# mateomarin/two_towers

Measured on AMD Instinct MI355X. Metric: training pairs/sec at global batch=8192, 1/2/4/8 GPUs; MRR@10 match, higher is better.
Workload: dtype bf16; 1 GPU; BASELINE configs[2]: EnhancedTwoTowerModel(300, 256), seq_len 64, batch 8192 per GPU, bf16, hard-negative mining k=5 + margin 0.2, dropout 0.1, Adam; global_batch=8192, seq_len=64, hidden=256, embedding_dim=300, parallelism=dp1, loss=hardneg_margin

## Files before the change

include/tt_hip.h:

```cpp
#ifndef TT_HIP_H
#define TT_HIP_H
#include <stdint.h>

#ifdef __cplusplus
extern "C" {
#endif

#define TT_OK 0
#define TT_EINVAL 1000
#define TT_DT_F32 0
#define TT_DT_BF16 1

const char* tt_version(void);
const char* tt_last_error(void);
int tt_set_option(const char* name, int value);
int tt_get_option(const char* name, int* value);

int tt_embed_gather(int dtype, const void* table, long vocab, int ep, const int32_t* ids, long n,
                    void* out, void* stream);

int tt_pack_rows(int dtype, const float* src, long n, int e, int ep, void* out, void* stream);
typedef struct {
  const float* src;
  const float* src2;
// ... 3 lines not shown
  int dst_bf16;
} tt_pack_job;
int tt_pack_multi(const tt_pack_job* jobs, int njobs, void* stream);

int tt_cast(int dtype, const float* x, long n, void* y, void* stream);

int tt_colsum(const float* x, long rows, int cols, long ld, float* out, int accumulate, void* stream);

typedef struct {
  const void* a[4];
  const void* b[4];
  void* c[4];
  const float* bias[4];
  int bshift[4];
  const void* a_hi[4];
  int a_split;
  uint32_t drop_row0;
} tt_gemm_batch;

int tt_gemm(int dtype, int out_dtype, int a_kouter, int b_kouter, int m, int n, int k,
            const tt_gemm_batch* batch, int nbatch, long lda, long ldb, long ldc, float alpha,
            int beta_accum, int relu, int seq_t, uint32_t drop_seed, float drop_p, int splits,
            float* splitk_ws, void* stream);
long tt_gemm_ws_size(int m, int n, int nbatch, int splits);
int tt_gemm_pick_splits(int m, int n, int k, int nbatch);
int tt_gemm_bres_form(int m, int n, int k, int nbatch, long lda, long ldc);

typedef struct {
  const void* g;
  const void* whh;
  const float* bhn;
  void* y;
  void* x1;
  void* save;
  float* hstate;
  int dir;
  uint32_t drop_seed;
  int drop_col0;
  uint32_t drop_row0;
} tt_gru_fwd_rec;

int tt_gru_fwd(int dtype, const tt_gru_fwd_rec* recs, int nrec, int B, int T, int H, long ldg,
               long ldy, float drop_p, void* ws, long ws_bytes, void* stream);
int tt_gru_fwd_launches(int dtype, int T, int H);
long tt_gru_fwd_ws_size(int dtype, int nrec, int B, int T, int H, long ldg, long ldy);
int tt_gru_fwd_launches_for(int dtype, int nrec, int B, int T, int H, long ldg, long ldy);

typedef struct {
  const void* g; const void* whh; const float* bhn;
// ... 120 lines not shown
```

two_towers_amd/_lib.py:

```python
from __future__ import annotations

import contextlib
import ctypes
import os
from ctypes import POINTER, c_float, c_int, c_long, c_uint32, c_void_p

import torch

_HERE = os.path.dirname(os.path.abspath(__file__))
LIB_PATH = os.environ.get("TT_HIP_LIB", os.path.join(_HERE, "lib", "libtt_hip.so"))

DT_F32 = 0
DT_BF16 = 1
TT_EINVAL = 1000


class TTError(RuntimeError):
    pass


class GruTimeoutError(TTError):
    """A column-split GRU forward launch gave up waiting for one of its member workgroups
    (tt_gru_fwd's status word): that launch's outputs are invalid."""

# ... 73 lines not shown


class Head1BwdIO(ctypes.Structure):
    _fields_ = [
        ("x", c_void_p), ("w1", c_void_p), ("ln_g", c_void_p), ("ln_b", c_void_p), ("p1", c_void_p),
        ("mean", c_void_p), ("rstd", c_void_p), ("dout", c_void_p), ("dx", c_void_p), ("dw1", c_void_p),
        ("db1", c_void_p), ("dg", c_void_p), ("dbeta", c_void_p), ("ws", c_void_p),
    ]


_SIGS = {
    "tt_version": (ctypes.c_char_p, []),
    "tt_last_error": (ctypes.c_char_p, []),
    "tt_set_option": (c_int, [ctypes.c_char_p, c_int]),
    "tt_get_option": (c_int, [ctypes.c_char_p, POINTER(c_int)]),
    "tt_embed_gather": (c_int, [c_int, c_void_p, c_long, c_int, c_void_p, c_long, c_void_p, c_void_p]),
    "tt_pack_rows": (c_int, [c_int, c_void_p, c_long, c_int, c_int, c_void_p, c_void_p]),
    "tt_pack_multi": (c_int, [c_void_p, c_int, c_void_p]),
    "tt_cast": (c_int, [c_int, c_void_p, c_long, c_void_p, c_void_p]),
    "tt_colsum": (c_int, [c_void_p, c_long, c_int, c_long, c_void_p, c_int, c_void_p]),
    "tt_gemm": (c_int, [c_int, c_int, c_int, c_int, c_int, c_int, c_int, POINTER(GemmBatch), c_int, c_long,
                        c_long, c_long, c_float, c_int, c_int, c_int, c_uint32, c_float, c_int, c_void_p,
                        c_void_p]),
    "tt_gemm_ws_size": (c_long, [c_int, c_int, c_int, c_int]),
    "tt_gemm_pick_splits": (c_int, [c_int, c_int, c_int, c_int]),
    "tt_gemm_bres_form": (c_int, [c_int, c_int, c_int, c_int, c_long, c_long]),
    "tt_gru_fwd": (c_int, [c_int, POINTER(GruFwdRec), c_int, c_int, c_int, c_int, c_long, c_long, c_float,
                           c_void_p, c_long, c_void_p]),
    "tt_gru_bwd": (c_int, [c_int, POINTER(GruBwdRec), c_int, c_int, c_int, c_int, c_long, c_long, c_long,
                           c_void_p]),
    "tt_gru_bias_rows": (c_int, [c_int]),
    "tt_gru_bwd_launches": (c_int, [c_int, c_int, c_int]),
    "tt_gru_bwd_carry_on_chip": (c_int, [c_int, c_int, c_int]),
    "tt_gru_fwd_launches": (c_int, [c_int, c_int, c_int]),
    "tt_gru_fwd_ws_size": (c_long, [c_int, c_int, c_int, c_int, c_int, c_long, c_long]),
    "tt_gru_fwd_launches_for": (c_int, [c_int, c_int, c_int, c_int, c_int, c_long, c_long]),
    "tt_gru_fwd_infer": (c_int, [c_int, POINTER(GruInferRec), c_int, c_int, c_int, c_int, c_long, c_long, c_long,
                                 c_void_p, c_long, c_void_p]),
    "tt_gru_infer_scratch_size": (c_long, [c_int, c_int, c_int, c_int, c_int]),
    "tt_proj_head_fwd": (c_int, [c_int, POINTER(HeadFwdIO), c_int, c_int, c_int, c_float, c_void_p]),
    "tt_proj_head_bwd": (c_int, [c_int, POINTER(HeadBwdIO), c_int, c_int, c_int, c_float, c_void_p]),
    "tt_proj_head_bwd_ws_size": (c_long, [c_int, c_int, c_int]),
    "tt_proj_head1_fwd": (c_int, [c_int, POINTER(Head1FwdIO), c_long, c_int, c_float, c_float, c_uint32,
                                  c_void_p]),
    "tt_proj_head1_bwd": (c_int, [c_int, POINTER(Head1BwdIO), c_long, c_int, c_float, c_uint32, c_void_p]),
    "tt_proj_head1_bwd_ws_size": (c_long, [c_int, c_long, c_int]),
    "tt_l2norm_fwd": (c_int, [c_int, c_void_p, c_long, c_int, c_float, c_void_p, c_void_p, c_void_p, c_void_p]),
    "tt_l2norm_bwd": (c_int, [c_void_p, c_void_p, c_void_p, c_long, c_int, c_float, c_void_p, c_int, c_void_p]),
    "tt_infonce_fwd": (c_int, [c_int, c_void_p, c_long, c_void_p, c_long, c_int, c_float, c_float, c_long,
# ... 108 lines not shown
```

two_towers_amd/csrc/tt_api.h:

```cpp
#pragma once
#include <hip/hip_runtime.h>
#include <stdio.h>
#include <string.h>

#include "../../include/tt_hip.h"

namespace tt {
void set_error(const char* fmt, ...);

enum Opt {
  OPT_GRU_STEP,
  OPT_GRU_DEPTH,
  OPT_GRU_BWD_ROWS,
  OPT_GRU_BWD_BIG,
  OPT_GRU_BWD_STREAMS,
  OPT_GEMM_PERSIST,
  OPT_GEMM_A3,
  OPT_GEMM_REGSTAGE,
  OPT_GEMM_STREAM_OUT,
  OPT_HN_GEMM,
  OPT_GRU_BWD_PERSIST,
  OPT_GRU_FWD_STEP_ROWS,
  OPT_INFONCE_FLASH,
  OPT_HN_MAP,
  OPT_GEMM_SKEW,
  OPT_GEMM_PERSIST_MAXK,
  OPT_GRU_FWD_XC,
  OPT_GRU_XC_SKIP,
  OPT_GRU_XC_SPINS,
  OPT_GRU_BWD_SKEW,
  OPT_GRU_FWD_SKEW,
  OPT_GEMM_BRES,
  OPT_GRU_XC_COOP,
  OPT_GEMM_BUF,
  OPT_GEMM_ORDER,
  OPT_GRU_STEP_RING,
  OPT_GRU_FWD_XS,
  OPT_HN_SCAN_GEMM,
  OPT_GEMM_IEPI,
  OPT_BRES_ROWS,
  OPT_HN_SCAN_V,
  OPT_GEMM_W4,
  OPT_BRES_FORM,
  OPT_N
};
int opt(Opt o);
int tt_hn_scan_gemm(const void* q, long bq, const void* d, long nd, int h, long label_off, float* cm, long nch,
                    hipStream_t st);
}

#define TT_CHECK_ARG(cond, ...)            \
  do {                                     \
    if (!(cond)) {                         \
      tt::set_error(__VA_ARGS__);          \
      return TT_EINVAL;                    \
    }                                      \
  } while (0)

#define TT_CHECK_LAUNCH(what)                                                        \
  do {                                                                               \
    hipError_t e_ = hipGetLastError();                                               \
    if (e_ != hipSuccess) {                                                          \
      tt::set_error("%s: %s", what, hipGetErrorString(e_));                          \
      return (int)e_;                                                                \
    }                                                                                \
  } while (0)
// ... 18 lines not shown
```

two_towers_amd/csrc/tt_gemm.hip:

```cpp
#include <float.h>
#include <stdarg.h>
#include <stdlib.h>

#include <atomic>
#include <type_traits>

#include "tt_api.h"
#include "tt_gemm_core.h"

namespace tt {
static thread_local char g_err[512];
void set_error(const char* fmt, ...) {
  va_list ap;
  va_start(ap, fmt);
  vsnprintf(g_err, sizeof(g_err), fmt, ap);
  va_end(ap);
}
}

namespace tt {
namespace {
struct OptDef {
  const char* name;
  const char* env;
  int dflt;
};
constexpr OptDef kOpts[OPT_N] = {
    {"gru_step", "TT_GRU_STEP", 0},               {"gru_depth", "TT_GRU_DEPTH", 4},
    {"gru_bwd_rows", "TT_GRU_BWD_ROWS", 0},     {"gru_bwd_big", "TT_GRU_BWD_BIG", 1},
    {"gru_bwd_streams", "TT_GRU_BWD_STREAMS", 2}, {"gemm_persist", "TT_GEMM_PERSIST", 1},
    {"gemm_a3", "TT_GEMM_A3", 1},                 {"gemm_regstage", "TT_GEMM_REGSTAGE", 0},
    {"gemm_stream_out", "TT_GEMM_STREAM_OUT", 1}, {"hn_gemm", "TT_HN_GEMM", 0},
    {"gru_bwd_persist", "TT_GRU_BWD_PERSIST", 1}, {"gru_fwd_step_rows", "TT_GRU_FWD_STEP_ROWS", 0},
    {"infonce_flash", "TT_INFONCE_FLASH", 1},     {"hn_map", "TT_HN_MAP", 2},
    {"gemm_skew", "TT_GEMM_SKEW", 0},             {"gemm_persist_maxk", "TT_GEMM_PERSIST_MAXK", 24},
    {"gru_fwd_xc", "TT_GRU_FWD_XC", 1},           {"gru_xc_skip", "TT_GRU_XC_SKIP", 0},
    {"gru_xc_spins", "TT_GRU_XC_SPINS", 22},      {"gru_bwd_skew", "TT_GRU_BWD_SKEW", 14},
    {"gru_fwd_skew", "TT_GRU_FWD_SKEW", 0},       {"gemm_bres", "TT_GEMM_BRES", 1},
    {"gru_xc_coop", "TT_GRU_XC_COOP", 0},         {"gemm_buf", "TT_GEMM_BUF", 1},
    {"gemm_order", "TT_GEMM_ORDER", 0},           {"gru_step_ring", "TT_GRU_STEP_RING", 4},
    {"gru_fwd_xs", "TT_GRU_FWD_XS", 1},           {"hn_scan_gemm", "TT_HN_SCAN_GEMM", 0},
    {"gemm_iepi", "TT_GEMM_IEPI", 1},             {"bres_rows", "TT_BRES_ROWS", 32},
    {"hn_scan_v", "TT_HN_SCAN_V", 5},             {"gemm_w4", "TT_GEMM_W4", 0},
    {"bres_form", "TT_BRES_FORM", 1},
};
struct OptTable {
  std::atomic<int> v[OPT_N];
  OptTable() {
    for (int i = 0; i < OPT_N; ++i) {
      const char* e = getenv(kOpts[i].env);
      v[i].store(e && *e ? atoi(e) : kOpts[i].dflt, std::memory_order_relaxed);
    }
  }
};
OptTable& opts() {
  static OptTable t;
  return t;
}
int find_opt(const char* name) {
  for (int i = 0; name && i < OPT_N; ++i)
    if (strcmp(name, kOpts[i].name) == 0) return i;
  return -1;
}
}
int opt(Opt o) { return opts().v[o].load(std::memory_order_relaxed); }
}

// ... 17 lines not shown
struct GemmArgs {
  const void* a[4];
  const void* b[4];
  void* c[4];
  const float* bias[4];
  int bshift[4];
  const void* a_hi[4];
  int a_split;
  long lda, ldb, ldc;
  int M, N, K;
  int splits, kt_per_split;
  float alpha;
  int beta, relu, seq_t;
  uint32_t drop_seed, drop_thresh, drop_row0;
  float drop_inv_keep;
  long part_stride;
  int vec_ok;
  int force_regstage;
  int skew;
  int bias_vec_ok;
  int stream_out;
  int walk_g, walk_x;
  int nbatch;
  float* cm;
  long nch, label_off;
};

constexpr int BM = 128, BN = 128;

#ifndef TT_TAIL_SKIP
#define TT_TAIL_SKIP 1
#endif
using ttg::xcd_remap;
#ifndef PERSIST_IEPI
#define PERSIST_IEPI 1
#endif
#ifndef PERSIST_BAL
#define PERSIST_BAL 1
#endif
#ifndef TT_EPI_PAIR
#define TT_EPI_PAIR 1
#endif
#ifndef TT_GEMM_BAL
#define TT_GEMM_BAL true
#endif

// ... 993 lines not shown
              st8(dst, v);
          } else {
            for (int e = 0; e < 8 && gn + e < g.N; ++e) Elt<TO>::st(dst + e, v[e]);
          }
        }
      }
      __builtin_amdgcn_s_barrier();
    }
    if (late && qn < qend) __builtin_amdgcn_s_barrier();
  }
  if constexpr (IE && A3 && !HN && PERSIST_BAL && std::is_same<TO, bf16_t>::value) {
    if (have_prev) {
      iepi(C0{}, C0{});
      iepi(C0{}, C1{});
      iepi(C1{}, C1{});
      iepi(C1{}, C0{});
    }
  }
  if constexpr (A3)
    if (!late) __builtin_amdgcn_s_barrier();
  asm volatile("s_waitcnt vmcnt(0)" ::: "memory");
}

template <typename TO, int V>
__global__ __launch_bounds__(256) void splitk_reduce_kernel(const float* ws, long part_stride, int splits,
                                                            int M, int N, GemmArgs g) {
  const int bi = blockIdx.y;
  const float* P = ws + (long)bi * splits * part_stride;
  TO* C = static_cast<TO*>(g.c[bi]);
  const float* bias = g.bias[bi];
  const long total = (long)M * N / V;
  for (long e = (long)blockIdx.x * 256 + threadIdx.x; e < total; e += (long)gridDim.x * 256) {
    float v[V];
    if constexpr (V == 4) {
      float4 a = make_float4(0.f, 0.f, 0.f, 0.f);
      for (int s = 0; s < splits; ++s) {
        const float4 b = reinterpret_cast<const float4*>(P + (long)s * part_stride)[e];
        a.x += b.x;
        a.y += b.y;
        a.z += b.z;
        a.w += b.w;
      }
      v[0] = a.x, v[1] = a.y, v[2] = a.z, v[3] = a.w;
    } else {
      v[0] = 0.f;
      for (int s = 0; s < splits; ++s) v[0] += P[(long)s * part_stride + e];
    }
    const int m = (int)(e * V / N), n0 = (int)(e * V % N);
#pragma unroll
    for (int u = 0; u < V; ++u) {
      float x = v[u] * g.alpha;
      if (bias) x += bias[n0 + u];
      TO* p = C + (long)m * g.ldc + n0 + u;
      if (g.beta) x += Elt<TO>::ld(p);
      Elt<TO>::st(p, x);
    }
  }
}

template <typename T, typename TO, int TBM, int TBN, int WGM, int WGN, bool DMA, bool A3 = false, bool BUF = false>
int launch_t(int akout, int bkout, bool shift, const GemmArgs& g, long nwg, hipStream_t st) {
  dim3 grid((unsigned)nwg), blk(64 * WGM * WGN);
#define TT_L(AK, BK, SH) \
  hipLaunchKernelGGL((gemm_kernel<T, AK, BK, SH, TO, TBM, TBN, WGM, WGN, DMA, A3, BUF>), grid, blk, 0, st, g)
  if (!akout && !bkout) TT_L(false, false, false);
  else if (!akout && bkout && !shift) TT_L(false, true, false);
  else if (!akout && bkout && shift) TT_L(false, true, true);
  else if (akout && !bkout) TT_L(true, false, false);
  else if (akout && bkout && !shift) TT_L(true, true, false);
  else TT_L(true, true, true);
#undef TT_L
  TT_CHECK_LAUNCH("gemm_kernel");
  return 0;
}

inline bool use_big(int m, int n, long tiles256) { return m >= 256 && n >= 256 && tiles256 >= 256; }
// ... 254 lines not shown
#define TT_WR(n)                                                                   \
  case n:                                                                          \
    if (form == 2)                                                                 \
      hipLaunchKernelGGL((gemm_wreg<n>), grid, blk, 0, st, g, npan, nbatch);       \
    else if (r64)                                                                  \
      hipLaunchKernelGGL((gemm_bres<n, 4>), grid, blk, 0, st, g, npan, nbatch);    \
    else                                                                           \
      hipLaunchKernelGGL((gemm_bres<n, 2>), grid, blk, 0, st, g, npan, nbatch);    \
    break;
      TT_WR(1) TT_WR(2) TT_WR(3) TT_WR(4) TT_WR(5) TT_WR(6) TT_WR(7) TT_WR(8) TT_WR(9) TT_WR(10) TT_BR(11) TT_BR(12)
#undef TT_WR
#undef TT_BR
      default: return false;
    }
    const hipError_t e = hipGetLastError();
    if (e != hipSuccess) {
      tt::set_error("%s: %s", form == 2 ? "gemm_wreg" : "gemm_bres", hipGetErrorString(e));
      *rc = (int)e;
    }
    return true;
  }
}

template <typename T, typename TO>
int launch_gemm(int akout, int bkout, bool shift, GemmArgs& g, int nbatch, hipStream_t st) {
  constexpr int EPC = 16 / (int)sizeof(T);
  {
    int rc = 0;
    if (try_bres<T, TO>(akout, bkout, shift, g, nbatch, st, &rc)) return rc;
  }
  const bool dma = (akout ? g.M % EPC == 0 : g.K % EPC == 0) && (bkout ? g.N % EPC == 0 : g.K % EPC == 0) &&
                   g.force_regstage != 1;
  const long t256 = (long)tt_ceil_div(g.M, 256) * tt_ceil_div(g.N, 256) * nbatch * g.splits;
  const bool persist_ok = tt::opt(tt::OPT_GEMM_PERSIST) != 0;
  const int nk = (g.K * (int)sizeof(T) + ttg::KTB - 1) / ttg::KTB;
  bool buf = tt::opt(tt::OPT_GEMM_BUF) != 0 && g.K % (ttg::KTB / (int)sizeof(T)) == 0;
  {
    const long span = (long)(g.kt_per_split + 2) * (ttg::KTB / (int)sizeof(T)) * (long)sizeof(T);
    if (akout && span * g.lda >= (1L << 32)) buf = false;
    if (bkout && span * g.ldb >= (1L << 32)) buf = false;
    if (shift && g.seq_t % (ttg::KTB / (int)sizeof(T)) != 0) buf = false;
    if (!akout && (long)256 * g.lda * (long)sizeof(T) >= (1L << 31)) buf = false;
    if (!bkout && (long)256 * g.ldb * (long)sizeof(T) >= (1L << 31)) buf = false;
    for (int b = 0; b < 4 && g.a_split > 0; ++b) {
      if (!g.a[b]) continue;
      const long d = (long)((const char*)g.a_hi[b] - (const char*)g.a[b]) / (long)sizeof(T);
      if (d < 0 || d + (g.M - g.a_split) > g.lda) buf = false;
    }
  }
  if constexpr (std::is_same<T, bf16_t>::value && std::is_same<TO, bf16_t>::value) {
    if (tt::opt(tt::OPT_GEMM_W4) && !akout && !bkout && !shift && g.splits == 1 && !g.beta && !g.relu &&
        !g.drop_thresh && g.alpha == 1.f && g.force_regstage == 0 && g.M % 256 == 0 && g.N % 256 == 0 && g.K % 64 == 0 &&
// ... 38 lines not shown
  g.alpha = 1.f;
  g.splits = 1;
  g.kt_per_split = h / 64;
  g.nbatch = 1;
  g.cm = cm;
  g.nch = nch;
  g.label_off = label_off;
  const long ntm = (bq + 255) / 256, ntn = (nd + 255) / 256, ntiles = ntm * ntn;
  TT_CHECK_ARG(ntiles < (1L << 31), "tt_hn_scan_gemm: too many tiles");
  if (ntiles % 256 == 0 && ntn % 4 == 0) {
    g.walk_g = 4;
    g.walk_x = 8;
  }
  hipLaunchKernelGGL((gemm_persist<bf16_t, false, false, false, float, true, true, true>),
                     dim3((unsigned)std::min<long>(ntiles, 256)), dim3(512), 0, st, g, (int)ntiles);
  TT_CHECK_LAUNCH("gemm_persist (hard-negative scan)");
  return 0;
}

extern "C" int tt_gemm_bres_form(int m, int n, int k, int nbatch, long lda, long ldc) {
  return bres_form_for(m, n, k, nbatch, lda, ldc);
}

extern "C" long tt_gemm_ws_size(int m, int n, int nbatch, int splits) {
  (void)m;
  return splits > 1 ? (long)m * n * nbatch * splits : 0;
}

extern "C" int tt_gemm_pick_splits(int m, int n, int k, int nbatch) {
  const bool big = m >= 256 && n >= 256;
  const long tiles = big ? (long)tt_ceil_div(m, 256) * tt_ceil_div(n, 256) * nbatch
                         : (long)tt_ceil_div(m, BM) * tt_ceil_div(n, BN) * nbatch;
  const long target = big ? 512 : 1024;
  if (tiles >= target) return 1;
  const int smax = std::max(1, std::min(64, tt_ceil_div(k, 64) / 8));
  int best = 1;
  double best_eff = 0.0;
  const int s_lo = (int)std::min<long>(smax, std::max<long>(1, target / tiles));
  for (int s = s_lo; s <= std::min<long>(smax, 3 * target / tiles + 1); ++s) {
    const long w = tiles * s;
    const double eff = (double)w / (256.0 * (double)tt_ceil_div(w, 256));
    if (eff > best_eff + 1e-9) { best_eff = eff; best = s; }
  }
  return std::min(best, smax);
}

extern "C" int tt_gemm(int dtype, int out_dtype, int a_kouter, int b_kouter, int m, int n, int k,
                       const tt_gemm_batch* batch, int nbatch, long lda, long ldb, long ldc,
                       float alpha, int beta_accum, int relu, int seq_t, uint32_t drop_seed,
                       float drop_p, int splits, float* splitk_ws, void* stream) {
  TT_CHECK_ARG(dtype == TT_DT_F32 || dtype == TT_DT_BF16, "tt_gemm: bad dtype %d", dtype);
  TT_CHECK_ARG(out_dtype == TT_DT_F32 || out_dtype == dtype, "tt_gemm: bad out_dtype %d", out_dtype);
  TT_CHECK_ARG(nbatch >= 1 && nbatch <= 4, "tt_gemm: nbatch %d not in [1,4]", nbatch);
  TT_CHECK_ARG(m >= 0 && n >= 0 && k >= 0, "tt_gemm: negative dims");
  if (m == 0 || n == 0) return 0;
  const int esz = dtype == TT_DT_BF16 ? 2 : 4;
  const int epc = 16 / esz;
  (void)epc;
  TT_CHECK_ARG((lda * esz) % 16 == 0 && (ldb * esz) % 16 == 0,
               "tt_gemm: leading dimensions must be 16-byte multiples (lda=%ld ldb=%ld)", lda, ldb);
  if (splits < 1) splits = 1;
  TT_CHECK_ARG(splits == 1 || (relu == 0 && drop_p == 0.f), "tt_gemm: split-K excludes relu/dropout");
  TT_CHECK_ARG(splits == 1 || splitk_ws != nullptr, "tt_gemm: split-K needs a workspace");
  TT_CHECK_ARG(drop_p >= 0.f && drop_p < 1.f, "tt_gemm: drop_p %f", drop_p);
  bool shift = false;
  GemmArgs g{};
  for (int b = 0; b < nbatch; ++b) {
    TT_CHECK_ARG(batch->a[b] && batch->b[b] && batch->c[b], "tt_gemm: null operand in batch %d", b);
    TT_CHECK_ARG(((uintptr_t)batch->a[b] | (uintptr_t)batch->b[b]) % 16 == 0,
                 "tt_gemm: operands must be 16-byte aligned (batch %d)", b);
    g.a[b] = batch->a[b];
    g.b[b] = batch->b[b];
    g.c[b] = batch->c[b];
    g.bias[b] = batch->bias[b];
    g.bshift[b] = batch->bshift[b];
    g.a_hi[b] = batch->a_hi[b];
    if (batch->a_split > 0)
      TT_CHECK_ARG(batch->a_hi[b] && (uintptr_t)batch->a_hi[b] % 16 == 0, "tt_gemm: a_hi[%d] null or misaligned", b);
    if (batch->bshift[b] != 0) shift = true;
  }
  TT_CHECK_ARG(!shift || (b_kouter && seq_t > 0), "tt_gemm: bshift needs b_kouter and seq_t");
  TT_CHECK_ARG(batch->a_split >= 0 && (batch->a_split == 0 || (a_kouter && batch->a_split % (16 / esz) == 0)),
               "tt_gemm: a_split %d needs a_kouter and a 16-byte multiple", batch->a_split);
  g.a_split = batch->a_split;
  g.lda = lda; g.ldb = ldb; g.ldc = ldc;
  g.M = m; g.N = n; g.K = k;
  g.alpha = alpha; g.beta = beta_accum; g.relu = relu; g.seq_t = seq_t;
  g.force_regstage = tt::opt(tt::OPT_GEMM_REGSTAGE);
  g.nbatch = nbatch;
  g.skew = tt::opt(tt::OPT_GEMM_SKEW);
  g.drop_seed = drop_seed;
  g.drop_row0 = batch->drop_row0;
  g.drop_thresh = drop_p > 0.f ? (uint32_t)(drop_p * 16777216.0f + 0.5f) : 0u;
  g.drop_inv_keep = drop_p > 0.f ? 1.0f / (1.0f - drop_p) : 1.0f;
  const int nk = tt_ceil_div((long)k * esz, 128);
  if (splits > nk) splits = nk > 0 ? nk : 1;
  g.kt_per_split = nk > 0 ? tt_ceil_div(nk, splits) : 1;
  splits = nk > 0 ? tt_ceil_div(nk, g.kt_per_split) : 1;
  g.splits = splits;
  {
    const int osz = out_dtype == TT_DT_BF16 ? 2 : 4;
    bool ok = (ldc * osz) % 16 == 0;
    for (int b = 0; b < nbatch; ++b) ok = ok && ((uintptr_t)batch->c[b] % 16 == 0);
    g.vec_ok = ok;
    bool bok = true;
    for (int b = 0; b < nbatch; ++b) bok = bok && ((uintptr_t)batch->bias[b] % 16 == 0);
    g.bias_vec_ok = bok;
    g.stream_out = ok && (long)m * n * osz >= (64L << 20) && (long)256 * ldc * osz < (1L << 31);
    g.stream_out = g.stream_out ? tt::opt(tt::OPT_GEMM_STREAM_OUT) : 0;
  }
  hipStream_t st = static_cast<hipStream_t>(stream);
  TT_CHECK_ARG((long)tt_ceil_div(m, 128) * tt_ceil_div(n, 128) * nbatch * splits < (1L << 31), "tt_gemm: too many tiles");

  if (splits > 1) {
    GemmArgs gp = g;
    gp.part_stride = (long)m * n;
    gp.vec_ok = (n % 4 == 0);
    for (int b = 0; b < nbatch; ++b) gp.c[b] = splitk_ws + (long)b * splits * gp.part_stride;
    int rc = dtype == TT_DT_BF16 ? launch_gemm<bf16_t, float>(a_kouter, b_kouter, shift, gp, nbatch, st)
                                 : launch_gemm<float, float>(a_kouter, b_kouter, shift, gp, nbatch, st);
    if (rc) return rc;
    const bool v4 = n % 4 == 0 && (uintptr_t)splitk_ws % 16 == 0;
// ... 19 lines not shown
```

two_towers_amd/csrc/tt_gemm_core.h:

```cpp
#pragma once
#include <type_traits>

#include "tt_common.h"

typedef __bf16 bf16x8v __attribute__((ext_vector_type(8)));
typedef short s16x4 __attribute__((ext_vector_type(4)));
typedef __attribute__((address_space(3))) s16x4 lds_s16x4;

#ifndef TT_PRIO_HALF
#define TT_PRIO_HALF 0
#endif
#ifndef TT_SHIFT_BUF
#define TT_SHIFT_BUF 1
#endif

namespace ttg {

constexpr int KTB = 128;

TT_DEV int kc_off(int row, int c) { return row * KTB + ((c ^ ((row >> 1) & 7)) << 4); }
TT_DEV int ko_v(int k) { return (k & 3) | (((k >> 3) & 1) << 2); }
TT_DEV int ko16_off(int k, int c) { return k * 256 + ((c ^ (ko_v(k) << 1)) << 4); }
TT_DEV int ko32_off_chunk(int k, int c) { return k * 512 + ((c ^ (((k >> 2) & 1) << 2)) << 4); }
TT_DEV int ko32_off_elem(int k, int m) { return k * 512 + ((m ^ (((k >> 2) & 1) << 4)) << 2); }

template <typename T, bool KO, int ROWS>
struct Img {
  static constexpr int BYTES = KO ? (KTB / (int)sizeof(T)) * ROWS * (int)sizeof(T) : ROWS * KTB;
  static constexpr int CHUNKS = BYTES / 16;
  static_assert(!KO || ROWS == 128, "K-outer images are 128 columns wide");
};


template <typename T>
TT_DEV uint4 load_partial(const T* p, int n) {
  union {
    uint4 v;
    T e[16 / sizeof(T)];
  } u;
  u.v = make_uint4(0, 0, 0, 0);
#pragma unroll
  for (int i = 0; i < (int)(16 / sizeof(T)); ++i)
    if (i < n) u.e[i] = p[i];
  return u.v;
}
// ... 59 lines not shown
    const int o0 = ko16_off(k0, cc >> 1) + ((cc & 1) << 3);
    const int o1 = ko16_off(k1, cc >> 1) + ((cc & 1) << 3);
    s16x4 lo = __builtin_amdgcn_ds_read_tr16_b64_v4i16((lds_s16x4*)(img + o0));
    s16x4 hi = __builtin_amdgcn_ds_read_tr16_b64_v4i16((lds_s16x4*)(img + o1));
    uint4 v;
    v.x = (uint32_t)(uint16_t)lo[0] | ((uint32_t)(uint16_t)lo[1] << 16);
    v.y = (uint32_t)(uint16_t)lo[2] | ((uint32_t)(uint16_t)lo[3] << 16);
    v.z = (uint32_t)(uint16_t)hi[0] | ((uint32_t)(uint16_t)hi[1] << 16);
    v.w = (uint32_t)(uint16_t)hi[2] | ((uint32_t)(uint16_t)hi[3] << 16);
    return v;
  } else {
    const int g = lane >> 4;
    const int m = r0 + (lane & 15);
    const int kb = ks * 16 + 4 * g;
    uint4 v;
    v.x = *reinterpret_cast<const uint32_t*>(img + ko32_off_elem(kb + 0, m));
    v.y = *reinterpret_cast<const uint32_t*>(img + ko32_off_elem(kb + 1, m));
    v.z = *reinterpret_cast<const uint32_t*>(img + ko32_off_elem(kb + 2, m));
    v.w = *reinterpret_cast<const uint32_t*>(img + ko32_off_elem(kb + 3, m));
    return v;
  }
}

template <typename T>
TT_DEV f32x4 mma(uint4 a, uint4 b, f32x4 c) {
  if constexpr (sizeof(T) == 2) {
    return __builtin_amdgcn_mfma_f32_16x16x32_bf16(__builtin_bit_cast(bf16x8v, a),
                                                   __builtin_bit_cast(bf16x8v, b), c, 0, 0, 0);
  } else {
    c = __builtin_amdgcn_mfma_f32_16x16x4f32(__uint_as_float(a.x), __uint_as_float(b.x), c, 0, 0, 0);
    c = __builtin_amdgcn_mfma_f32_16x16x4f32(__uint_as_float(a.y), __uint_as_float(b.y), c, 0, 0, 0);
    c = __builtin_amdgcn_mfma_f32_16x16x4f32(__uint_as_float(a.z), __uint_as_float(b.z), c, 0, 0, 0);
    c = __builtin_amdgcn_mfma_f32_16x16x4f32(__uint_as_float(a.w), __uint_as_float(b.w), c, 0, 0, 0);
    return c;
  }
}

template <typename T, bool AKO, bool BKO, int BM, int BN>
struct MainLoop {
  using IA = Img<T, AKO, BM>;
  using IB = Img<T, BKO, BN>;
  static constexpr int STAGE = IA::BYTES + IB::BYTES;
  static constexpr int LDS_BYTES = 2 * STAGE;
  static constexpr int TM = BM / 32, TN = BN / 32;
  static_assert(IA::CHUNKS % 256 == 0 && IB::CHUNKS % 256 == 0, "tile/thread mismatch");

// ... 748 lines not shown
```

two_towers_amd/ops.py:

```python
from __future__ import annotations

import ctypes
from typing import Sequence

import torch

from . import _lib
from ._lib import GemmBatch, call, dtype_code, ptr, stream_ptr


def _esz(dt: torch.dtype) -> int:
    return 2 if dt == torch.bfloat16 else 4


def pad_cols(e: int, dt: torch.dtype) -> int:
    epc = 128 // _esz(dt)
    return (e + epc - 1) // epc * epc


def gemm(a: Sequence[torch.Tensor], b: Sequence[torch.Tensor], c: Sequence[torch.Tensor], *, m: int, n: int,
         k: int, lda: int, ldb: int, ldc: int, a_kouter: bool, b_kouter: bool, dtype: torch.dtype,
         out_dtype: torch.dtype, bias: Sequence[torch.Tensor | None] | None = None,
         bshift: Sequence[int] | None = None, alpha: float = 1.0, accumulate: bool = False,
         relu: bool = False, seq_t: int = 0, drop_seed: int = 0, drop_p: float = 0.0, drop_row0: int = 0,
         splits: int | None = None, a_hi: Sequence[torch.Tensor] | None = None, a_split: int = 0):
    nb = len(a)
    assert 1 <= nb <= 4 and len(b) == nb and len(c) == nb
    bt = GemmBatch()
    for i in range(nb):
        assert a[i].dtype == dtype and b[i].dtype == dtype, (a[i].dtype, b[i].dtype, dtype)
        assert c[i].dtype == out_dtype, (c[i].dtype, out_dtype)
        bt.a[i] = a[i].data_ptr()
        bt.b[i] = b[i].data_ptr()
        bt.c[i] = c[i].data_ptr()
        bt.bias[i] = bias[i].data_ptr() if bias is not None and bias[i] is not None else None
        bt.bshift[i] = bshift[i] if bshift is not None else 0
        if a_split:
            bt.a_hi[i] = a_hi[i].data_ptr()
    bt.a_split = a_split
    bt.drop_row0 = drop_row0 & 0xFFFFFFFF
    lib = _lib.load()
    if splits is None:
        splits = lib.tt_gemm_pick_splits(m, n, k, nb)
    ws = None
    if splits > 1 and not relu and drop_p == 0.0:
        ws = torch.empty(lib.tt_gemm_ws_size(m, n, nb, splits), dtype=torch.float32, device=c[0].device)
    else:
        splits = 1
    call("tt_gemm", dtype_code(dtype), dtype_code(out_dtype), int(a_kouter), int(b_kouter), m, n, k,
         ctypes.byref(bt), nb, lda, ldb, ldc, alpha, int(accumulate), int(relu), seq_t, drop_seed & 0xFFFFFFFF,
         drop_p, splits, ptr(ws), stream_ptr(c[0].device))


def embed_gather(table: torch.Tensor, ids: torch.Tensor, out: torch.Tensor):
    assert ids.dtype == torch.int32 and ids.is_contiguous()
    assert table.dim() == 2 and out.shape[-1] == table.shape[1] and out.dtype == table.dtype
    call("tt_embed_gather", dtype_code(table.dtype), table.data_ptr(), table.shape[0], table.shape[1],
         ids.data_ptr(), ids.numel(), out.data_ptr(), stream_ptr(out.device))


def pack_rows(src: torch.Tensor, out: torch.Tensor):
    assert src.dtype == torch.float32 and src.is_contiguous()
    e = src.shape[-1]
    n = src.numel() // e
    call("tt_pack_rows", dtype_code(out.dtype), src.data_ptr(), n, e, out.shape[-1], out.data_ptr(),
         stream_ptr(out.device))


def cast(x: torch.Tensor, out: torch.Tensor):
    assert x.dtype == torch.float32 and x.is_contiguous() and out.numel() == x.numel()
    call("tt_cast", dtype_code(out.dtype), x.data_ptr(), x.numel(), out.data_ptr(), stream_ptr(out.device))


def colsum(x: torch.Tensor, rows: int, cols: int, ld: int, out: torch.Tensor, accumulate: bool = False):
# ... 30 lines not shown
```

two_towers_amd/towers.py:

```python
from __future__ import annotations

import ctypes
import os
import threading
from dataclasses import dataclass

import torch
import torch.nn.functional as F

from . import _lib, dist, ops, timing
from ._lib import GruBwdRec, GruFwdRec, GruInferRec, HeadBwdIO, HeadFwdIO, call, dtype_code, stream_ptr

PARAMS_PER_TOWER = 22
LN_EPS = 1e-5
HEAD_DT = torch.float32


def gru_param_names():
    names = []
    for layer in (0, 1):
        for sfx in ("", "_reverse"):
            for w in ("weight_ih", "weight_hh", "bias_ih", "bias_hh"):
                names.append(f"{w}_l{layer}{sfx}")
    return names
# ... 406 lines not shown


def _weight_grads(cfg, B, T, dG, Xin, K, ldx, Y, kr=None):
    n, H, dt, dev = cfg.ntowers, cfg.H, cfg.dtype, dG[0].device
    BT = B * T
    dWih = [[_alloc((3 * H, K), torch.float32, dev) for _ in range(2)] for _ in range(n)]
    dWhh = [[_alloc((3 * H, H), torch.float32, dev) for _ in range(2)] for _ in range(n)]
    a_ih, b_ih, c_ih, a_hh, a_hi, b_hh, c_hh, sh = [], [], [], [], [], [], [], []
    for ti in range(n):
        for d in range(2):
            a_ih.append(dG[ti][:, d * 3 * H:])
            b_ih.append(Xin[ti])
            c_ih.append(dWih[ti][d])
            a_hh.append(dG[ti][:, d * 3 * H:])
            a_hi.append(dG[ti][:, 6 * H + d * H:])
            b_hh.append(Y[ti][:, d * H:])
            c_hh.append(dWhh[ti][d])
            sh.append(-1 if d == 0 else 1)
    esz = 2 if dt == torch.bfloat16 else 4
    kr = K if kr is None else kr
    with timing.region("wgrad_ih", 1, 2.0 * 3 * H * kr * BT * 2 * n,
                       float(n * (esz * BT * (6 * H + kr) + 2 * 3 * H * kr * 4))):
        if _WGRAD_T and dt == torch.bfloat16 and 0 < K % 256 <= 128:
            cT = [_alloc((K, 3 * H), torch.float32, dev) for _ in c_ih]
            ops.gemm(b_ih, a_ih, cT, m=K, n=3 * H, k=BT, lda=ldx, ldb=8 * H, ldc=3 * H, a_kouter=True,
                     b_kouter=True, dtype=dt, out_dtype=torch.float32)
            for c, ct in zip(c_ih, cT):
                c.copy_(ct.t())
        else:
            ops.gemm(a_ih, b_ih, c_ih, m=3 * H, n=K, k=BT, lda=8 * H, ldb=ldx, ldc=K, a_kouter=True,
                     b_kouter=True, dtype=dt, out_dtype=torch.float32)
    with timing.region("wgrad_hh", 1, 2.0 * 3 * H * H * BT * 2 * n,
                       float(n * (esz * BT * (6 * H + 2 * H) + 2 * 3 * H * H * 4))):
        ops.gemm(a_hh, b_hh, c_hh, m=3 * H, n=H, k=BT, lda=8 * H, ldb=2 * H, ldc=H, a_kouter=True, b_kouter=True,
                 dtype=dt, out_dtype=torch.float32, bshift=sh, seq_t=T, a_hi=a_hi, a_split=2 * H)
    return dWih, dWhh


class TowersFn(torch.autograd.Function):

    @staticmethod
    def forward(ctx, cfg: TowerCfg, table, group, cache_ok, *args):
        n = cfg.ntowers
        xs, params = args[:n], args[n:]
        _lib.require_gpu(*xs, *params)
        check_gru_status(wait=True)
        dt, E, H, h = cfg.dtype, cfg.E, cfg.H, cfg.h
        dev = xs[0].device
        reset_guard_if_reported(dev)
        B, T = xs[0].shape[0], xs[0].shape[1]
        for x in xs:
# ... 179 lines not shown
```

Baseline: 155,800 pairs/s.

## Add tall-M wgrad GEMM kernel and transposed split-K reduce output

New measurement: 157,400 pairs/s, median of 6. +1.1%, better.

```diff
diff --git a/include/tt_hip.h b/include/tt_hip.h
--- a/include/tt_hip.h
+++ b/include/tt_hip.h
@@ -49,9 +49,15 @@
             const tt_gemm_batch* batch, int nbatch, long lda, long ldb, long ldc, float alpha,
             int beta_accum, int relu, int seq_t, uint32_t drop_seed, float drop_p, int splits,
             float* splitk_ws, void* stream);
+int tt_gemm_ct(int dtype, int out_dtype, int a_kouter, int b_kouter, int m, int n, int k,
+               const tt_gemm_batch* batch, int nbatch, long lda, long ldb, long ldc, float alpha,
+               int beta_accum, int relu, int seq_t, uint32_t drop_seed, float drop_p, int splits,
+               float* splitk_ws, int c_trans, void* stream);
 long tt_gemm_ws_size(int m, int n, int nbatch, int splits);
 int tt_gemm_pick_splits(int m, int n, int k, int nbatch);
 int tt_gemm_bres_form(int m, int n, int k, int nbatch, long lda, long ldc);
+int tt_gemm_tall_form(int dtype, int out_dtype, int a_kouter, int b_kouter, int m, int n, int k, long lda,
+                      long ldb, int splits, int extras);
 
 typedef struct {
   const void* g;
diff --git a/two_towers_amd/_lib.py b/two_towers_amd/_lib.py
--- a/two_towers_amd/_lib.py
+++ b/two_towers_amd/_lib.py
@@ -119,9 +119,13 @@
     "tt_gemm": (c_int, [c_int, c_int, c_int, c_int, c_int, c_int, c_int, POINTER(GemmBatch), c_int, c_long,
                         c_long, c_long, c_float, c_int, c_int, c_int, c_uint32, c_float, c_int, c_void_p,
                         c_void_p]),
+    "tt_gemm_ct": (c_int, [c_int, c_int, c_int, c_int, c_int, c_int, c_int, POINTER(GemmBatch), c_int, c_long,
+                           c_long, c_long, c_float, c_int, c_int, c_int, c_uint32, c_float, c_int, c_void_p,
+                           c_int, c_void_p]),
     "tt_gemm_ws_size": (c_long, [c_int, c_int, c_int, c_int]),
     "tt_gemm_pick_splits": (c_int, [c_int, c_int, c_int, c_int]),
     "tt_gemm_bres_form": (c_int, [c_int, c_int, c_int, c_int, c_long, c_long]),
+    "tt_gemm_tall_form": (c_int, [c_int, c_int, c_int, c_int, c_int, c_int, c_int, c_long, c_long, c_int, c_int]),
     "tt_gru_fwd": (c_int, [c_int, POINTER(GruFwdRec), c_int, c_int, c_int, c_int, c_long, c_long, c_float,
                            c_void_p, c_long, c_void_p]),
     "tt_gru_bwd": (c_int, [c_int, POINTER(GruBwdRec), c_int, c_int, c_int, c_int, c_long, c_long, c_long,
diff --git a/two_towers_amd/csrc/tt_api.h b/two_towers_amd/csrc/tt_api.h
--- a/two_towers_amd/csrc/tt_api.h
+++ b/two_towers_amd/csrc/tt_api.h
@@ -42,6 +42,7 @@
   OPT_HN_SCAN_V,
   OPT_GEMM_W4,
   OPT_BRES_FORM,
+  OPT_WGRAD_TALL,
   OPT_N
 };
 int opt(Opt o);
diff --git a/two_towers_amd/csrc/tt_gemm.hip b/two_towers_amd/csrc/tt_gemm.hip
--- a/two_towers_amd/csrc/tt_gemm.hip
+++ b/two_towers_amd/csrc/tt_gemm.hip
@@ -42,7 +42,7 @@
     {"gru_fwd_xs", "TT_GRU_FWD_XS", 1},           {"hn_scan_gemm", "TT_HN_SCAN_GEMM", 0},
     {"gemm_iepi", "TT_GEMM_IEPI", 1},             {"bres_rows", "TT_BRES_ROWS", 32},
     {"hn_scan_v", "TT_HN_SCAN_V", 5},             {"gemm_w4", "TT_GEMM_W4", 0},
-    {"bres_form", "TT_BRES_FORM", 1},
+    {"bres_form", "TT_BRES_FORM", 1},             {"wgrad_tall", "TT_WGRAD_TALL", 1},
 };
 struct OptTable {
   std::atomic<int> v[OPT_N];
@@ -106,6 +106,7 @@
   int stream_out;
   int walk_g, walk_x;
   int nbatch;
+  int c_trans;
   float* cm;
   long nch, label_off;
 };
@@ -1145,6 +1146,140 @@
   asm volatile("s_waitcnt vmcnt(0)" ::: "memory");
 }
 
+namespace tall {
+constexpr int AW = 8192, AN = 4096;
+constexpr int BOFF = 2 * AW + AN;
+constexpr int SLOT = BOFF + 2 * AW;
+constexpr int NS = 4;
+constexpr int NDMA = SLOT / 1024;
+constexpr int KS = 32;
+}
+
+template <bool HALF>
+__global__ __launch_bounds__(512) void gemm_tall(GemmArgs g, int u0) {
+  using namespace tall;
+  constexpr int NA = HALF ? 5 : 10;
+  __shared__ __attribute__((aligned(16))) char lds[NS * SLOT];
+  const int ntn = (g.N + 255) / 256;
+  const int id = xcd_remap(blockIdx.x, gridDim.x);
+  const int hf = HALF ? id & 1 : 0;
+  const int u = u0 + (HALF ? id >> 1 : id);
+  const int bs = u / ntn, nt = u - bs * ntn;
+  const int bi = bs / g.splits, s = bs - bi * g.splits;
+  const int n0 = nt * 256;
+  const bf16_t* A = static_cast<const bf16_t*>(g.a[bi]);
+  const bf16_t* B = static_cast<const bf16_t*>(g.b[bi]);
+  const int wave = __builtin_amdgcn_readfirstlane(threadIdx.x >> 6), lane = threadIdx.x & 63;
+  const int wr = wave >> 2, wn = (wave & 3) * 64;
+  auto a_sub = [&](int a) { return HALF ? a >> 1 : a / 5; };
+  auto a_col = [&](int a) {
+    if (HALF) return a == 4 ? 32 * hf + 16 * wr : 64 * hf + 32 * wr + 16 * (a & 1);
+    return a % 5 == 4 ? 32 * wr + 16 * (a / 5) : 64 * wr + 16 * (a % 5);
+  };
+
+  f32x4 acc[NA][4];
+#pragma unroll
+  for (int i = 0; i < NA; ++i)
+#pragma unroll
+    for (int j = 0; j < 4; ++j) acc[i][j] = f32x4{0.f, 0.f, 0.f, 0.f};
+
+  const int nk = (g.K * 2 + ttg::KTB - 1) / ttg::KTB;
+  const int kt0 = s * g.kt_per_split;
+  const int kt1 = min(nk, kt0 + g.kt_per_split);
+  if (kt0 < kt1) {
+    const int nst = 2 * (kt1 - kt0);
+    const long k0 = (long)kt0 * 64;
+    const long krows = min((long)g.K, (long)kt1 * 64) - k0;
+    const ttg::tt_rsrc4 ra = ttg::make_rsrc4(A + k0 * g.lda, (uint32_t)(((krows - 1) * g.lda + g.M) * 2));
+    const ttg::tt_rsrc4 rb = ttg::make_rsrc4(B + k0 * g.ldb, (uint32_t)(((krows - 1) * g.ldb + g.N) * 2));
+    const uint32_t da = (uint32_t)(KS * g.lda * 2), db = (uint32_t)(KS * g.ldb * 2);
+    uint32_t voff[5];
+#pragma unroll
+    for (int t = 0; t < 5; ++t) {
+      const int j = wave + 8 * t;
+      long e;
+      if (j < 16) {
+        const int p = (j & 7) * 64 + lane, kl = p >> 4, c = (p & 15) ^ (ttg::ko_v(kl) << 1);
+        e = (long)kl * g.lda + (j >> 3) * 128 + c * 8;
+      } else if (j < 20) {
+        const int p = (j - 16) * 64 + lane, kl = p >> 3, c = (p & 7) ^ (ttg::kon_v(kl) << 1);
+        e = (long)kl * g.lda + 256 + c * 8;
+      } else {
+        const int b = j - 20, p = (b & 7) * 64 + lane, kl = p >> 4, c = (p & 15) ^ (ttg::ko_v(kl) << 1);
+        e = (long)kl * g.ldb + n0 + (b >> 3) * 128 + c * 8;
+      }
+      voff[t] = (uint32_t)(e * 2);
+    }
+    const uint32_t base = __builtin_amdgcn_readfirstlane(ttg::lds_addr_of(lds));
+    const bool a2 = wave < 4;
+    ttg::tt_rsrc4 r2;
+    r2.x = a2 ? ra.x : rb.x;
+    r2.y = a2 ? ra.y : rb.y;
+    r2.z = a2 ? ra.z : rb.z;
+    r2.w = ra.w;
+    const uint32_t d2 = a2 ? da : db;
+    auto issue = [&](int st) {
+      const uint32_t sl = base + (uint32_t)(st & (NS - 1)) * SLOT + (uint32_t)wave * 1024u;
+      const uint32_t sa = (uint32_t)st * da, sb = (uint32_t)st * db;
+      ttg::dma16_buf(ra, voff[0] + sa, 0u, sl);
+      ttg::dma16_buf(ra, voff[1] + sa, 0u, sl + 8 * 1024u);
+      ttg::dma16_buf(r2, voff[2] + (uint32_t)st * d2, 0u, sl + 16 * 1024u);
+      ttg::dma16_buf(rb, voff[3] + sb, 0u, sl + 24 * 1024u);
+      if (a2) ttg::dma16_buf(rb, voff[4] + sb, 0u, sl + 32 * 1024u);
+    };
+    auto step = [&](const char* sl) {
+      uint4 fb[4];
+#pragma unroll
+      for (int j = 0; j < 4; ++j) fb[j] = ttg::frag<bf16_t, true>(sl + BOFF + (wn >> 7) * AW, (wn & 127) + 16 * j, 0);
+#pragma unroll
+      for (int h = 0; h < NA / 5; ++h) {
+        uint4 fa[5];
+#pragma unroll
+        for (int i = 0; i < 4; ++i) fa[i] = ttg::frag<bf16_t, true>(sl + a_sub(5 * h + i) * AW, a_col(5 * h + i), 0);
+        fa[4] = ttg::frag_ko16n(sl + 2 * AW, a_col(5 * h + 4));
+#pragma unroll
+        for (int i = 0; i < 5; ++i)
+#pragma unroll
+          for (int j = 0; j < 4; ++j) acc[5 * h + i][j] = ttg::mma<bf16_t>(fb[j], fa[i], acc[5 * h + i][j]);
+        __builtin_amdgcn_sched_barrier(0);
+      }
+    };
+    issue(0);
+    issue(1);
+    issue(2);
+    for (int st = 0; st < nst; ++st) {
+      if (wave < 4) asm volatile("s_waitcnt vmcnt(10)" ::: "memory");
+      else asm volatile("s_waitcnt vmcnt(8)" ::: "memory");
+      __builtin_amdgcn_s_barrier();
+      issue(st + 3);
+      const char* sl = lds + (st & (NS - 1)) * SLOT;
+      step(sl);
+    }
+    asm volatile("s_waitcnt vmcnt(0)" ::: "memory");
+  }
+
+  const bool partial = g.splits > 1;
+  float* C = partial ? static_cast<float*>(g.c[bi]) + (long)s * g.part_stride : static_cast<float*>(g.c[bi]);
+  const long ldc = partial ? (long)g.N : g.ldc;
+  const int q = lane >> 4, lr = lane & 15;
+#pragma unroll
+  for (int i = 0; i < NA; ++i) {
+    const int gm = (i % 5 < 4 ? 128 * a_sub(i) : 256) + a_col(i) + lr;
+#pragma unroll
+    for (int j = 0; j < 4; ++j) {
+      const int c = n0 + wn + 16 * j + 4 * q;
+      if (gm >= g.M || c >= g.N) continue;
+      float v[4];
+#pragma unroll
+      for (int e = 0; e < 4; ++e) v[e] = partial ? acc[i][j][e] : acc[i][j][e] * g.alpha + 0.f;
+      float* dst = C + (long)gm * ldc + c;
+      if (c + 4 <= g.N && g.vec_ok) *reinterpret_cast<float4*>(dst) = make_float4(v[0], v[1], v[2], v[3]);
+      else
+        for (int e = 0; e < 4 && c + e < g.N; ++e) dst[e] = v[e];
+    }
+  }
+}
+
 template <typename TO, int V>
 __global__ __launch_bounds__(256) void splitk_reduce_kernel(const float* ws, long part_stride, int splits,
                                                             int M, int N, GemmArgs g) {
@@ -1174,7 +1309,7 @@
     for (int u = 0; u < V; ++u) {
       float x = v[u] * g.alpha;
       if (bias) x += bias[n0 + u];
-      TO* p = C + (long)m * g.ldc + n0 + u;
+      TO* p = g.c_trans ? C + (long)(n0 + u) * g.ldc + m : C + (long)m * g.ldc + n0 + u;
       if (g.beta) x += Elt<TO>::ld(p);
       Elt<TO>::st(p, x);
     }
@@ -1475,12 +1610,40 @@
   }
 }
 
+bool tall_form_for(bool bf16_in, bool f32_out, int akout, int bkout, bool plain, int M, int N, long lda, long ldb,
+                   int kt_per_split) {
+  if (tt::opt(tt::OPT_WGRAD_TALL) == 0 || !bf16_in || !f32_out || !akout || !bkout || !plain) return false;
+  if (M <= 256 || M > 320 || M % 8 || N % 8 || N <= 0) return false;
+  if (tt::opt(tt::OPT_GEMM_REGSTAGE) != 0) return false;
+  const long span = ((long)kt_per_split * 64 + 4 * tall::KS) * 2;
+  return span * lda < (1L << 32) && span * ldb < (1L << 32);
+}
+bool gemm_args_plain(const GemmArgs& g, bool shift, int nbatch) {
+  if (shift || g.a_split > 0 || g.beta || g.relu || g.drop_thresh) return false;
+  for (int b = 0; b < nbatch; ++b)
+    if (g.bias[b]) return false;
+  return true;
+}
+
 template <typename T, typename TO>
 int launch_gemm(int akout, int bkout, bool shift, GemmArgs& g, int nbatch, hipStream_t st) {
   constexpr int EPC = 16 / (int)sizeof(T);
   {
     int rc = 0;
     if (try_bres<T, TO>(akout, bkout, shift, g, nbatch, st, &rc)) return rc;
+  }
+  if (tall_form_for(std::is_same<T, bf16_t>::value, std::is_same<TO, float>::value, akout, bkout,
+                    gemm_args_plain(g, shift, nbatch), g.M, g.N, g.lda, g.ldb, g.kt_per_split)) {
+    const long units = (long)tt_ceil_div(g.N, 256) * nbatch * g.splits;
+    const int mode = tt::opt(tt::OPT_WGRAD_TALL);
+    long nfull = units;
+    if (mode == 3) nfull = 0;
+    else if (mode != 2 && units % 256 > 0 && units % 256 <= 128) nfull = units - units % 256;
+    if (nfull > 0) hipLaunchKernelGGL(gemm_tall<false>, dim3((unsigned)nfull), dim3(512), 0, st, g, 0);
+    if (units > nfull)
+      hipLaunchKernelGGL(gemm_tall<true>, dim3((unsigned)(2 * (units - nfull))), dim3(512), 0, st, g, (int)nfull);
+    TT_CHECK_LAUNCH("gemm_tall");
+    return 0;
   }
   const bool dma = (akout ? g.M % EPC == 0 : g.K % EPC == 0) && (bkout ? g.N % EPC == 0 : g.K % EPC == 0) &&
                    g.force_regstage != 1;
@@ -1565,6 +1728,23 @@
   return bres_form_for(m, n, k, nbatch, lda, ldc);
 }
 
+static void split_plan(int k, int esz, int* splits, int* kt_per_split) {
+  const int nk = tt_ceil_div((long)k * esz, 128);
+  int s = *splits < 1 ? 1 : *splits;
+  if (s > nk) s = nk > 0 ? nk : 1;
+  *kt_per_split = nk > 0 ? tt_ceil_div(nk, s) : 1;
+  *splits = nk > 0 ? tt_ceil_div(nk, *kt_per_split) : 1;
+}
+
+extern "C" int tt_gemm_tall_form(int dtype, int out_dtype, int a_kouter, int b_kouter, int m, int n, int k, long lda,
+                                 long ldb, int splits, int extras) {
+  int ktps = 1;
+  split_plan(k, dtype == TT_DT_BF16 ? 2 : 4, &splits, &ktps);
+  return tall_form_for(dtype == TT_DT_BF16, out_dtype == TT_DT_F32, a_kouter, b_kouter, extras == 0, m, n, lda, ldb, ktps)
+             ? 1
+             : 0;
+}
+
 extern "C" long tt_gemm_ws_size(int m, int n, int nbatch, int splits) {
   (void)m;
   return splits > 1 ? (long)m * n * nbatch * splits : 0;
@@ -1592,6 +1772,14 @@
                        const tt_gemm_batch* batch, int nbatch, long lda, long ldb, long ldc,
                        float alpha, int beta_accum, int relu, int seq_t, uint32_t drop_seed,
                        float drop_p, int splits, float* splitk_ws, void* stream) {
+  return tt_gemm_ct(dtype, out_dtype, a_kouter, b_kouter, m, n, k, batch, nbatch, lda, ldb, ldc, alpha, beta_accum, relu,
+                    seq_t, drop_seed, drop_p, splits, splitk_ws, 0, stream);
+}
+
+extern "C" int tt_gemm_ct(int dtype, int out_dtype, int a_kouter, int b_kouter, int m, int n, int k,
+                          const tt_gemm_batch* batch, int nbatch, long lda, long ldb, long ldc,
+                          float alpha, int beta_accum, int relu, int seq_t, uint32_t drop_seed,
+                          float drop_p, int splits, float* splitk_ws, int c_trans, void* stream) {
   TT_CHECK_ARG(dtype == TT_DT_F32 || dtype == TT_DT_BF16, "tt_gemm: bad dtype %d", dtype);
   TT_CHECK_ARG(out_dtype == TT_DT_F32 || out_dtype == dtype, "tt_gemm: bad out_dtype %d", out_dtype);
   TT_CHECK_ARG(nbatch >= 1 && nbatch <= 4, "tt_gemm: nbatch %d not in [1,4]", nbatch);
@@ -1636,11 +1824,10 @@
   g.drop_row0 = batch->drop_row0;
   g.drop_thresh = drop_p > 0.f ? (uint32_t)(drop_p * 16777216.0f + 0.5f) : 0u;
   g.drop_inv_keep = drop_p > 0.f ? 1.0f / (1.0f - drop_p) : 1.0f;
-  const int nk = tt_ceil_div((long)k * esz, 128);
-  if (splits > nk) splits = nk > 0 ? nk : 1;
-  g.kt_per_split = nk > 0 ? tt_ceil_div(nk, splits) : 1;
-  splits = nk > 0 ? tt_ceil_div(nk, g.kt_per_split) : 1;
+  split_plan(k, esz, &splits, &g.kt_per_split);
   g.splits = splits;
+  TT_CHECK_ARG(!c_trans || splits > 1, "tt_gemm_ct: a transposed C needs split-K (splits %d)", splits);
+  g.c_trans = c_trans != 0;
   {
     const int osz = out_dtype == TT_DT_BF16 ? 2 : 4;
     bool ok = (ldc * osz) % 16 == 0;
diff --git a/two_towers_amd/csrc/tt_gemm_core.h b/two_towers_amd/csrc/tt_gemm_core.h
--- a/two_towers_amd/csrc/tt_gemm_core.h
+++ b/two_towers_amd/csrc/tt_gemm_core.h
@@ -21,6 +21,8 @@
 TT_DEV int kc_off(int row, int c) { return row * KTB + ((c ^ ((row >> 1) & 7)) << 4); }
 TT_DEV int ko_v(int k) { return (k & 3) | (((k >> 3) & 1) << 2); }
 TT_DEV int ko16_off(int k, int c) { return k * 256 + ((c ^ (ko_v(k) << 1)) << 4); }
+TT_DEV int kon_v(int k) { return ((k >> 1) & 1) | (((k >> 3) & 1) << 1); }
+TT_DEV int ko16n_off(int k, int c) { return k * 128 + ((c ^ (kon_v(k) << 1)) << 4); }
 TT_DEV int ko32_off_chunk(int k, int c) { return k * 512 + ((c ^ (((k >> 2) & 1) << 2)) << 4); }
 TT_DEV int ko32_off_elem(int k, int m) { return k * 512 + ((m ^ (((k >> 2) & 1) << 4)) << 2); }
 
@@ -126,6 +128,23 @@
   }
 }
 
+TT_DEV uint4 frag_ko16n(const char* img, int r0) {
+  const int lane = threadIdx.x & 63;
+  const int g = lane >> 4, i4 = lane & 15, q = i4 >> 2, p = i4 & 3;
+  const int k0 = 8 * g + q;
+  const int cc = (r0 >> 2) + p;
+  const int o0 = ko16n_off(k0, cc >> 1) + ((cc & 1) << 3);
+  const int o1 = ko16n_off(k0 + 4, cc >> 1) + ((cc & 1) << 3);
+  s16x4 lo = __builtin_amdgcn_ds_read_tr16_b64_v4i16((lds_s16x4*)(img + o0));
+  s16x4 hi = __builtin_amdgcn_ds_read_tr16_b64_v4i16((lds_s16x4*)(img + o1));
+  uint4 v;
+  v.x = (uint32_t)(uint16_t)lo[0] | ((uint32_t)(uint16_t)lo[1] << 16);
+  v.y = (uint32_t)(uint16_t)lo[2] | ((uint32_t)(uint16_t)lo[3] << 16);
+  v.z = (uint32_t)(uint16_t)hi[0] | ((uint32_t)(uint16_t)hi[1] << 16);
+  v.w = (uint32_t)(uint16_t)hi[2] | ((uint32_t)(uint16_t)hi[3] << 16);
+  return v;
+}
+
 template <typename T>
 TT_DEV f32x4 mma(uint4 a, uint4 b, f32x4 c) {
   if constexpr (sizeof(T) == 2) {
diff --git a/two_towers_amd/ops.py b/two_towers_amd/ops.py
--- a/two_towers_amd/ops.py
+++ b/two_towers_amd/ops.py
@@ -23,7 +23,8 @@
          out_dtype: torch.dtype, bias: Sequence[torch.Tensor | None] | None = None,
          bshift: Sequence[int] | None = None, alpha: float = 1.0, accumulate: bool = False,
          relu: bool = False, seq_t: int = 0, drop_seed: int = 0, drop_p: float = 0.0, drop_row0: int = 0,
-         splits: int | None = None, a_hi: Sequence[torch.Tensor] | None = None, a_split: int = 0):
+         splits: int | None = None, a_hi: Sequence[torch.Tensor] | None = None, a_split: int = 0,
+         c_trans: bool = False):
     nb = len(a)
     assert 1 <= nb <= 4 and len(b) == nb and len(c) == nb
     bt = GemmBatch()
@@ -41,15 +42,24 @@
     bt.drop_row0 = drop_row0 & 0xFFFFFFFF
     lib = _lib.load()
     if splits is None:
-        splits = lib.tt_gemm_pick_splits(m, n, k, nb)
+        splits = gemm_splits(m, n, k, nb, dtype)
     ws = None
     if splits > 1 and not relu and drop_p == 0.0:
         ws = torch.empty(lib.tt_gemm_ws_size(m, n, nb, splits), dtype=torch.float32, device=c[0].device)
     else:
         splits = 1
-    call("tt_gemm", dtype_code(dtype), dtype_code(out_dtype), int(a_kouter), int(b_kouter), m, n, k,
+    call("tt_gemm_ct", dtype_code(dtype), dtype_code(out_dtype), int(a_kouter), int(b_kouter), m, n, k,
          ctypes.byref(bt), nb, lda, ldb, ldc, alpha, int(accumulate), int(relu), seq_t, drop_seed & 0xFFFFFFFF,
-         drop_p, splits, ptr(ws), stream_ptr(c[0].device))
+         drop_p, splits, ptr(ws), int(c_trans), stream_ptr(c[0].device))
+
+
+def gemm_splits(m: int, n: int, k: int, nb: int, dtype: torch.dtype) -> int:
+    s = _lib.load().tt_gemm_pick_splits(m, n, k, nb)
+    nk = (k * _esz(dtype) + 127) // 128
+    if nk <= 0:
+        return 1
+    per = (nk + min(max(s, 1), nk) - 1) // min(max(s, 1), nk)
+    return (nk + per - 1) // per
 
 
 def embed_gather(table: torch.Tensor, ids: torch.Tensor, out: torch.Tensor):
diff --git a/two_towers_amd/towers.py b/two_towers_amd/towers.py
--- a/two_towers_amd/towers.py
+++ b/two_towers_amd/towers.py
@@ -452,11 +452,15 @@
     with timing.region("wgrad_ih", 1, 2.0 * 3 * H * kr * BT * 2 * n,
                        float(n * (esz * BT * (6 * H + kr) + 2 * 3 * H * kr * 4))):
         if _WGRAD_T and dt == torch.bfloat16 and 0 < K % 256 <= 128:
-            cT = [_alloc((K, 3 * H), torch.float32, dev) for _ in c_ih]
-            ops.gemm(b_ih, a_ih, cT, m=K, n=3 * H, k=BT, lda=ldx, ldb=8 * H, ldc=3 * H, a_kouter=True,
-                     b_kouter=True, dtype=dt, out_dtype=torch.float32)
-            for c, ct in zip(c_ih, cT):
-                c.copy_(ct.t())
+            if ops.gemm_splits(K, 3 * H, BT, len(c_ih), dt) > 1:
+                ops.gemm(b_ih, a_ih, c_ih, m=K, n=3 * H, k=BT, lda=ldx, ldb=8 * H, ldc=K, a_kouter=True,
+                         b_kouter=True, dtype=dt, out_dtype=torch.float32, c_trans=True)
+            else:
+                cT = [_alloc((K, 3 * H), torch.float32, dev) for _ in c_ih]
+                ops.gemm(b_ih, a_ih, cT, m=K, n=3 * H, k=BT, lda=ldx, ldb=8 * H, ldc=3 * H, a_kouter=True,
+                         b_kouter=True, dtype=dt, out_dtype=torch.float32)
+                for c, ct in zip(c_ih, cT):
+                    c.copy_(ct.t())
         else:
             ops.gemm(a_ih, b_ih, c_ih, m=3 * H, n=K, k=BT, lda=8 * H, ldb=ldx, ldc=K, a_kouter=True,
                      b_kouter=True, dtype=dt, out_dtype=torch.float32)
```
